# artiom-matvei/RLAO

Measured on AMD Instinct MI355X. Metric: AO env-steps/sec (batched loops), higher is better.
Workload: dtype f32; 1 GPU; 8m / 20x20 Shack-Hartmann, 256 batched envs per GPU, integrator closed loop (BASELINE.json configs[1]); envs_per_gpu=256, envs_total=256, resolution=120, n_valid_act=357, n_signal=632, layers=1, controller=leaky integrator, gain 0.5, noise=photon, parallelism=env-shards x1, all-gather of episode returns

## Files before the change

### rlao_amd/csrc/common.hpp

```cpp
#pragma once
#include <hip/hip_runtime.h>
#include <stdint.h>
#include <stddef.h>

#include <string>
#include <vector>

#include "aoenv.h"

namespace ao {

constexpr int kWave = 64;
constexpr int kMaxLayer = 8;
constexpr int kMtN = 624;
constexpr int kMaxSplits = 16;
constexpr int kMaxModes = 512;

int fail(const char* fmt, ...);
#define AO_HIP(call)                                                                          \
    do {                                                                                      \
        hipError_t e_ = (call);                                                               \
        if (e_ != hipSuccess)                                                                 \
            return ::ao::fail("%s:%d: %s -> %s", __FILE__, __LINE__, #call, hipGetErrorString(e_)); \
    } while (0)
// ... 35 lines not shown
#pragma clang fp contract(off)
    for (int d = 0; d < 2; ++d) buff[d] += fmod(fabs(ratio[d]), 1.0) * clock_sgn(ratio[d]);
    *bx = fabs(buff[0]) < 1 ? 0 : (int)clock_sgn(buff[0]);
    *by = fabs(buff[1]) < 1 ? 0 : (int)clock_sgn(buff[1]);
    for (int d = 0; d < 2; ++d) buff[d] = fmod(fabs(buff[d]), 1.0) * clock_sgn(buff[d]);
    return *bx != 0 || *by != 0;
}

__host__ __device__ inline int clock_rounds(const double ratio[2], int j, int* sx, int* sy) {
#pragma clang fp contract(off)
    const int nx = (int)fabs(ratio[0]), ny = (int)fabs(ratio[1]);
    const int mn = nx < ny ? nx : ny, mx = nx > ny ? nx : ny;
    const int s0 = (int)clock_sgn(ratio[0]), s1 = (int)clock_sgn(ratio[1]);
    if (j < mn) {
        *sx = s0;
        *sy = s1;
    } else if (j < mx) {
        *sx = nx == mn ? 0 : s0;
        *sy = ny == mn ? 0 : s1;
    } else {
        *sx = *sy = 0;
    }
    return mx;
}

__host__ __device__ inline void clock_rounds_origin(const double ratio[2], int j, int S, int org[2]) {
#pragma clang fp contract(off)
    const int nx = (int)fabs(ratio[0]), ny = (int)fabs(ratio[1]);
    const int cx = (j < nx ? j : nx) * (int)clock_sgn(ratio[0]), cy = (j < ny ? j : ny) * (int)clock_sgn(ratio[1]);
    org[0] = ((org[0] - cy) % S + S) % S;
    org[1] = ((org[1] - cx) % S + S) % S;
}

__host__ __device__ inline void taps_from_buff(const double buff[2], LayerTaps& t) {
#pragma clang fp contract(off)
    const double fy = -buff[1], fx = -buff[0];
    const double ky = floor(fy), kx = floor(fx);
    t.dy = (int)ky;
    t.dx = (int)kx;
    catmull_rom(fy - ky, t.wy);
    catmull_rom(fx - kx, t.wx);
}

struct PhaseArgs {
    const void* screen[kMaxLayer];
    const void* minmax[kMaxLayer];
    LayerTaps taps[kMaxLayer];
    int n_layer;
    int S;
    int foot;
    int S_l[kMaxLayer];
    int foot_l[kMaxLayer];
    int update_atm;
    int store_atm;
    int store_phase;
    int minmax_dirty[kMaxLayer];
    const LayerTaps* env_taps;
    int n_env;
};

__device__ inline const LayerTaps& layer_taps(const PhaseArgs& pa, int l, int e) {
    return pa.env_taps ? pa.env_taps[(size_t)l * pa.n_env + e] : pa.taps[l];
}

__device__ inline double wave_sum_f64(double v) {
    for (int off = 32; off > 0; off >>= 1) v += __shfl_down(v, off);
// ... 10 lines not shown
int launch_ring_prepare(const T* map, T* zx, const int* inner_idx, const uint32_t* mt_state, const int* mt_pos,
                        uint32_t* mt_state_out, int* mt_pos_out, const int* env_idx, int n, int S, int n_inner, int n_outer, int K,
                        int sx, int sy, int oy, int ox, const double* xi_scale, hipStream_t st);
template <typename T>
int launch_mt_normal(uint32_t* mt_state, int* mt_pos, T* zx, int n_env, int K, int n_inner, int n_outer,
                     const double* xi_scale, hipStream_t st);
template <typename T>
int launch_scatter_minmax(T* new_map, const T* X, const int* outer_idx, T* minmax, const int* env_idx, int n, int n_env, int S,
                          int n_outer, int splits, int oy, int ox, int with_minmax, hipStream_t st, const LayerTaps* env_taps = nullptr);
template <typename T>
int launch_ring_prepare_env(const T* map, T* zx, const int* inner_idx, uint32_t* mt_state, int* mt_pos, const EnvClock* clk_in,
                            EnvClock* clk_out, LayerTaps* taps, double weight, int n_env, int S, int n_inner, int n_outer, int K,
                            const double* xi_scale, hipStream_t st);
template <typename T>
int launch_ring_round_env(const T* map, T* zx, const int* inner_idx, uint32_t* mt_state, int* mt_pos, const EnvClock* clk,
                          LayerTaps* taps, int j, int n_env, int S, int n_inner, int n_outer, int K, const double* xi_scale,
                          hipStream_t st);
template <typename T>
int launch_minmax(const T* maps, T* minmax, int n_env, int S, hipStream_t st);
int launch_mt_seed(const uint32_t* seeds, int stride, const int* env_idx, uint32_t* mt_state, int* mt_pos, int n, hipStream_t st);
template <typename T>
int launch_reset_env_rows(const int* env_idx, int n_idx, T* coefs, T* dm_prev, int n_valid_act, EnvClock* clk, LayerTaps* taps,
                          int n_layer, int n_env, hipStream_t st);
int gemm_splits(int M, int N, int K);
struct MtAhead {
    const uint32_t* mt_in;
    const int* pos_in;
    uint32_t* mt_out;
    int* pos_out;
    float* zx_out;
    int K, n_inner, n_outer, n_env;
    const double* xi_scale;
};
int launch_ring_gemm_draw_ahead(const float* X, const float* W, float* Cpart, int M, int N, int K, int splits, const MtAhead& m,
                                hipStream_t st);
int launch_sum_slabs(float* x, size_t n, int slabs, hipStream_t st);
int launch_gemm_nt_mfma(const float* X, const float* W, float* Cpart, int M, int N, int K, int ldx, int ldw, int splits,
                        hipStream_t st, int xsplits = 1, size_t xslab = 0);
template <typename T>
int launch_gemm_nt(const T* X, const T* W, T* C, int M, int N, int K, int ldx, int ldw, int ldc, hipStream_t st);

__host__ __device__ inline size_t ga_index(int x, int k, int ga_stride) {
    const int q = k & 3, s = k >> 2;
    return ((((size_t)(x >> 4) * (ga_stride >> 2) + (s >> 2)) * 4 + q) * 16 + (x & 15)) * 4 + (s & 3);
}
template <typename T>
struct PhaseBuffers {
    T* opd_atm;
    const T* coefs;
    const T* coefs_img;
    const T* dm_opd;
    const T* gx;
    const T* gy;
    const T* gxt;
    const float* gxa;
    const float* gya;
    int ga_stride;
    size_t g_env, gxt_env, ga_env;
    const float* s1a;
    const int* act_idx;
    const uint8_t* pupil;
    T* phase;
    double* part;
    T* wfs_max;
};
int phase_tiles(int R, int n_act, size_t esz);
template <typename T>
int launch_coefs_image(const T* coefs, const int* act_idx, T* img, int n_env, int n_act, int n_valid_act, hipStream_t st);
// ... 68 lines not shown
                   int max_group, hipStream_t st);
struct DetectorCfg {
    int active;
    int photon_noise, bits, emccd;
    float qe, dark_e, fwc, gain, readout_noise;
    uint32_t seed_lo, seed_hi;
    uint32_t frame_counter;
    uint32_t env_offset;
};

}
#include "poisson_alias.hpp"
namespace ao {

struct StepArgs {
    KArgs<float> k;
    ShConst<float> sc;
    FinishArgs<float> fa;
    float* frame;
    int store_phase, store_frame;
    float* signal;
    float* wfs_max;
    const float* fac_m;
    const float* fac_m2c_t;
    const short* slot_of;
    const float* amp_pupil;
    const float* gxa;
    const float* gya;
    size_t ga_env;
    DetectorCfg det;
    PoissonAlias pa;
    const float* ring_x[kMaxLayer];
    int ring_splits[kMaxLayer];
    const int* outer_idx;
    int n_outer;
    float* next_zx[kMaxLayer];
    int next_sx[kMaxLayer], next_sy[kMaxLayer];
    const int* inner_idx;
    int n_inner, zx_ld;
    int n_modes, n_subap, n_valid, n_env;
};
int step_fused_supported(int R, int n_subap, int n_valid, int n_act, int n_modes);
int step_alias_capacity(int n_act);
int launch_env_step(const StepArgs& a, const StarEnv<float>& star, hipStream_t st);

template <typename T>
struct RolloutActionArgs {
    const T* obs;
    T* action;
    const T* fr;
    const T* fl_t;
    const int* act_slot;
    const T* sigma_env;
    T gain, sigma;
    int n_act, n_valid_act, n_filter;
    uint32_t seed_lo, seed_hi, counter, env_offset;
};
constexpr size_t kRolloutLdsMax = 160 * 1024;
size_t rollout_action_lds(int n_valid_act, int n_filter, size_t esz);
template <typename T>
int launch_rollout_action(const RolloutActionArgs<T>& a, int n_env, hipStream_t st);

template <typename T>
struct DisturbArgs {
    const T* coefs;
    T* seen;
// ... 142 lines not shown
```

### rlao_amd/csrc/env.hip

```cpp
#include <algorithm>
#include <cmath>
#include <cstdarg>
#include <cstdio>
#include <cstring>
#include <initializer_list>
#include <new>
#include <utility>

#include "common.hpp"
#include "delay.hpp"
#include "dm_tables.hpp"
#include "detector.hpp"
#include "disturb.hpp"
#include "modal.hpp"
#include "policy.hpp"
#include "sh_device.hpp"
#include "science.hpp"
#include "star_env.hpp"
#include "wavefront.hpp"

namespace ao {

static thread_local std::string g_err;

int fail(const char* fmt, ...) {
    char buf[1024];
    va_list ap;
    va_start(ap, fmt);
    vsnprintf(buf, sizeof(buf), fmt, ap);
    va_end(ap);
    g_err = buf;
    return 1;
}

struct LayerClock {
    double ratio[2] = {0, 0};
    double buff[2] = {0, 0};
};

struct RingAhead { bool valid = false; int sx = 0, sy = 0, buf = 0; };

struct Layer {
    int N = 0, S = 0, nin = 0, nout = 0, K = 0;
    size_t scr_off = 0;
    void* ab = nullptr;
    int* inner_idx = nullptr;
    int* outer_idx = nullptr;
    bool have_ab = false, have_in = false, have_out = false;
    double weight = 0;
    LayerClock clk;
    int org[2] = {0, 0};
    uint32_t* mt_cur = nullptr;
    int* pos_cur = nullptr;
    uint32_t* mt_alt = nullptr;
    int* pos_alt = nullptr;
    int ring_pending = 0;
    const void* ring_src = nullptr;
    RingAhead ahead;
    bool gather_next = false;
    bool minmax_dirty = false;
    int env_rounds = 0;
};

}

using namespace ao;

struct AoEnv {
    AoCfg c{};
    int device = 0;
    size_t esz = 4;
    int R = 0, A = 0, nAct = 0, E = 0, L = 0, nSig = 0, nSub = 0, nVal = 0;
    int p = 0, n = 0, n_pupil = 0;
    Layer layer[kMaxLayer];
    size_t scr_elems = 0;
    int Kmax = 0, noutmax = 0, Smax = 0;
    bool uniform = true;
    int last_zx_layer = 0;
    bool per_env_wind = false;
    EnvClock* env_clk[2] = {nullptr, nullptr};
    int clk_cur = 0;
    int wind_pixels = 1;
    LayerTaps* env_taps = nullptr;
    bool per_env_r0 = false;
    std::vector<double> h_r0;
    double* xi_scale = nullptr;
    const double* sigma() const { return per_env_r0 ? xi_scale : nullptr; }
    bool use_coefs_img = false;
    bool defer_ring = true;
    bool have[AOENV_C_COUNT] = {false};
    double units = 1.0;
    void* screen = nullptr;
    void* minmax = nullptr;
    void* zx_pipe = nullptr;
    const void* last_zx = nullptr;
    bool use_lookahead = true;
    void* zx = nullptr;
    void* xbuf = nullptr;
    void* gx = nullptr;
    void* gy = nullptr;
    void* gxt = nullptr;
    void* modes = nullptr;
    void* dm_opd = nullptr;
    int* act_idx = nullptr;
    uint8_t* pupil = nullptr;
    void* opd_atm = nullptr;
    void* coefs = nullptr;
    void* dm_prev = nullptr;
    void* coefs_seen = nullptr;
    void* step_cmd = nullptr;
    void* cmd() const { return step_cmd ? step_cmd : coefs; }
    struct Disturb {
        bool set = false;
        int M = 0, J = 0;
        int64_t t0 = 0;
        void* modes_t = nullptr;
        double* par = nullptr;
        size_t modes_cap = 0, par_cap = 0;
    } disturb;
    DelayLine delay;
    void* delay_ring = nullptr;
    size_t delay_stride = 0;
    void* delay_slot(int slot) const { return static_cast<char*>(delay_ring) + (size_t)slot * delay_stride * esz; }
    struct Modal {
        bool set = false, have_gain = false;
        int K = 0;
        size_t gain_env = 0;
// ... 94 lines not shown
    int noise_K = 0;
    std::vector<int32_t> h_act_idx;
    int* act_slot = nullptr;
    bool act_slot_dirty = true;
    void* rollout_scratch = nullptr;
    uint32_t explore_counter = 0;
    uint64_t explore_seed = 0;
    bool explore_seeded = false;
    struct Policy {
        bool set = false, mfma = false;
        int H = 0, F = 0, Kp = 0;
        double slope = 0, clamp_abs = 0, b3 = 0;
        void *w1 = nullptr, *b1 = nullptr, *w2 = nullptr, *b2 = nullptr, *w3 = nullptr, *wt1 = nullptr, *wt2 = nullptr;
        void *proj_fr = nullptr, *proj_fl_t = nullptr, *hid1 = nullptr, *hid2 = nullptr;
    } policy;
    std::vector<void*> allocs;
    bool use_fast_wfs = true;
    bool use_mfma = true;
    bool use_fast_trig = true;
    bool use_fused_tail = true;
    bool use_fused_step = true;
    bool store_opd_atm = false;
    bool atm_user_defined = false;
    int force_path = 0;
    bool prof_on = false;
    struct ProfEv { int stage; hipEvent_t a, b; };
    std::vector<ProfEv> prof_ev;

    template <typename T> T* as(void* p_) const { return static_cast<T*>(p_); }
    void* screen_ptr(int l) const { return static_cast<char*>(screen) + layer[l].scr_off * esz; }
    void* minmax_ptr(int l) const { return static_cast<char*>(minmax) + (size_t)l * E * 2 * esz; }
    void* xbuf_ptr(int l) const { return static_cast<char*>(xbuf) + (size_t)l * kMaxSplits * E * noutmax * esz; }
    void* zx_pipe_ptr(int buf, int l) const { return static_cast<char*>(zx_pipe) + ((size_t)buf * L + l) * E * Kmax * esz; }
};

namespace {

int dmalloc(AoEnv* env, void** p, size_t bytes, bool zero = true);
static int alloc_dm_rows(AoEnv* env) {
    if (env->esz == 4 && env->nAct <= 128) {
        if (!env->dm_rows)
            AO_TRY(dmalloc(env, (void**)&env->dm_rows, (size_t)env->E * (cdiv(env->R, 128) * 128) * 4 * env->ga_stride * sizeof(float)));
    } else if (!env->coefs_img) {
        AO_TRY(dmalloc(env, &env->coefs_img, (size_t)env->E * env->nAct * env->nAct * env->esz));
    }
    return 0;
}
int dmalloc(AoEnv* env, void** p, size_t bytes, bool zero) {
    if (bytes == 0) bytes = 16;
    AO_HIP(hipMalloc(p, bytes));
    env->allocs.push_back(*p);
    if (zero) AO_HIP(hipMemset(*p, 0, bytes));
    return 0;
}

struct ProfScope {
    AoEnv* env; hipStream_t st; hipEvent_t a = nullptr, b = nullptr; int stage;
    ProfScope(AoEnv* e, int stage_, hipStream_t s) : env(e), st(s), stage(stage_) {
        if (!env->prof_on) return;
        if (hipEventCreate(&a) != hipSuccess || hipEventCreate(&b) != hipSuccess) { a = b = nullptr; return; }
        (void)hipEventRecord(a, st);
    }
    ~ProfScope() {
        if (!a) return;
        (void)hipEventRecord(b, st);
        env->prof_ev.push_back({stage, a, b});
// ... 19 lines not shown
ShConst<T> sh_const(const AoEnv* env) {
    ShConst<T> sc;
    sc.amp = env->as<T>(env->amp);
    sc.subap_idx = env->subap_idx;
    sc.valid2d = env->use_fast_wfs ? env->valid2d : nullptr;
    sc.ref = env->as<T>(env->sh_ref);
    sc.tw = env->as<T>(env->tw);
    sc.ph = env->as<T>(env->phs);
    sc.units = (T)env->units;
    sc.threshold = (T)env->c.threshold_cog;
    sc.fast_trig = (env->use_fast_trig && sizeof(T) == 4) ? 1 : 0;
    sc.plain = (env->force_path & AOENV_PATH_SH_PLAIN) ? 1 : 0;
    return sc;
}

template <typename T>
int gemm_dispatch(AoEnv* env, const T* X, const T* W, T* C, int M, int N, int K, int* splits, hipStream_t st);
template <>
int gemm_dispatch<float>(AoEnv* env, const float* X, const float* W, float* C, int M, int N, int K, int* splits,
                         hipStream_t st) {
    if (!env->use_mfma) { *splits = 1; return launch_gemm_nt<float>(X, W, C, M, N, K, K, K, N, st); }
    *splits = gemm_splits(M, N, K);
    return launch_gemm_nt_mfma(X, W, C, M, N, K, K, K, *splits, st);
}
template <>
int gemm_dispatch<double>(AoEnv*, const double* X, const double* W, double* C, int M, int N, int K, int* splits,
                          hipStream_t st) {
    *splits = 1;
    return launch_gemm_nt<double>(X, W, C, M, N, K, K, K, N, st);
}

void forget_lookahead(Layer& y) { y.ahead.valid = false; y.gather_next = false; }

void drop_ring(Layer& y) { y.ring_pending = 0; }

void move_origin(Layer& y, int sx, int sy) {
    y.org[0] = ((y.org[0] - sy) % y.S + y.S) % y.S;
    y.org[1] = ((y.org[1] - sx) % y.S + y.S) % y.S;
}

void defer_ring(AoEnv* env, int l, const void* zx, int splits) {
    env->last_zx = zx;
    env->last_zx_layer = l;
    env->layer[l].ring_pending = splits;
    env->layer[l].ring_src = env->xbuf_ptr(l);
}

void take_rings(AoEnv* env, StepArgs& a) {
    for (int l = 0; l < env->L; ++l) {
        Layer& y = env->layer[l];
        a.ring_x[l] = y.ring_pending ? static_cast<const float*>(y.ring_src) : nullptr;
        a.ring_splits[l] = y.ring_pending;
        const bool g = y.gather_next && y.ring_pending && y.ahead.valid;
        a.next_zx[l] = g ? static_cast<float*>(env->zx_pipe_ptr(y.ahead.buf, l)) : nullptr;
        a.next_sx[l] = y.ahead.sx;
        a.next_sy[l] = y.ahead.sy;
        if (y.gather_next && !g) y.ahead.valid = false;
        y.gather_next = false;
    }
}

void rings_written(AoEnv* env) {
    for (int l = 0; l < env->L; ++l) { env->layer[l].ring_pending = 0; env->layer[l].minmax_dirty = false; }
}

template <typename T>
int scatter_ring(AoEnv* env, int l, const LayerTaps* et, bool with_minmax, hipStream_t st) {
    Layer& y = env->layer[l];
    AO_PROF(env, SCATTER, st);
    AO_TRY(launch_scatter_minmax<T>(env->as<T>(env->screen_ptr(l)), static_cast<const T*>(y.ring_src), y.outer_idx,
                                    env->as<T>(env->minmax_ptr(l)), nullptr, env->E, env->E, y.S, y.nout, y.ring_pending, y.org[0],
                                    y.org[1], with_minmax ? 1 : 0, st, et));
    y.ring_pending = 0;
    return 0;
}

template <typename T>
int flush_ring(AoEnv* env, int l, hipStream_t st) {
    Layer& y = env->layer[l];
    if (!y.ring_pending) return 0;
    if (y.gather_next) forget_lookahead(y);
    const LayerTaps* et = env->per_env_wind ? env->env_taps + (size_t)l * env->E : nullptr;
    return scatter_ring<T>(env, l, et, et != nullptr, st);
}
template <typename T>
int flush_rings(AoEnv* env, hipStream_t st) {
    for (int l = 0; l < env->L; ++l) AO_TRY(flush_ring<T>(env, l, st));
    return 0;
}

template <typename T>
int ring_gemm(AoEnv* env, int l, const T* zx, int* splits, hipStream_t st) {
    const Layer& y = env->layer[l];
    AO_PROF(env, GEMM_RING, st);
    return gemm_dispatch<T>(env, zx, env->as<T>(y.ab), env->as<T>(env->xbuf_ptr(l)), env->E, y.nout, y.K, splits, st);
}

template <typename T>
int extrude(AoEnv* env, int l, int sx, int sy, bool lean, hipStream_t st, bool defer = false) {
    Layer& y = env->layer[l];
    forget_lookahead(y);
    AO_TRY(flush_ring<T>(env, l, st));
    T* zx = env->as<T>(env->zx);
    {
        AO_PROF(env, SHIFT_GATHER, st);
        AO_TRY(launch_ring_prepare<T>(env->as<T>(env->screen_ptr(l)), zx, y.inner_idx, y.mt_cur, y.pos_cur, y.mt_cur, y.pos_cur, nullptr,
// ... 30 lines not shown
    if (!d_idx) y.minmax_dirty = false;
    return 0;
}

template <typename T>
int refresh_minmax(AoEnv* env, hipStream_t st) {
    AO_TRY(flush_rings<T>(env, st));
    for (int l = 0; l < env->L; ++l)
        if (env->layer[l].minmax_dirty) {
            AO_TRY(launch_minmax<T>(env->as<T>(env->screen_ptr(l)), env->as<T>(env->minmax_ptr(l)), env->E, env->layer[l].S, st));
            env->layer[l].minmax_dirty = false;
        }
    return 0;
}

bool next_crossing(const LayerClock& k0, int* sx, int* sy) {
    if ((int)std::fabs(k0.ratio[0]) > 0 || (int)std::fabs(k0.ratio[1]) > 0) return false;
    if (k0.ratio[0] == 0 && k0.ratio[1] == 0) return false;
    double b[2] = {k0.buff[0], k0.buff[1]};
    for (int it = 0; it < 1000000; ++it) {
        for (int d = 0; d < 2; ++d) b[d] += std::fmod(std::fabs(k0.ratio[d]), 1.0) * sgn(k0.ratio[d]);
        if (std::fabs(b[0]) >= 1 || std::fabs(b[1]) >= 1) {
            *sx = std::fabs(b[0]) < 1 ? 0 : (int)sgn(b[0]);
            *sy = std::fabs(b[1]) < 1 ? 0 : (int)sgn(b[1]);
            return true;
        }
        for (int d = 0; d < 2; ++d) b[d] = std::fmod(std::fabs(b[d]), 1.0) * sgn(b[d]);
    }
    return false;
}

int extrude_pipelined(AoEnv* env, int l, int sx, int sy, hipStream_t st) {
    Layer& y = env->layer[l];
    const int cur = y.ahead.buf;
    float* op = static_cast<float*>(env->zx_pipe_ptr(cur, l));
    if (y.ahead.valid && y.ahead.sx == sx && y.ahead.sy == sy) {
        std::swap(y.mt_cur, y.mt_alt);
        std::swap(y.pos_cur, y.pos_alt);
    } else {
        AO_PROF(env, SHIFT_GATHER, st);
        AO_TRY(launch_ring_prepare<float>(env->as<float>(env->screen_ptr(l)), op, y.inner_idx, y.mt_cur, y.pos_cur, y.mt_cur, y.pos_cur,
                                          nullptr, env->E, y.S, y.nin, y.nout, y.K, sx, sy, y.org[0], y.org[1], env->sigma(), st));
    }
    forget_lookahead(y);
    const int splits = gemm_splits(env->E, y.nout, y.K);
    MtAhead m{y.mt_cur, y.pos_cur, y.mt_alt, y.pos_alt, static_cast<float*>(env->zx_pipe_ptr(1 - cur, l)), y.K, y.nin, y.nout, env->E,
              env->sigma()};
    {
        AO_PROF(env, GEMM_RING, st);
        AO_TRY(launch_ring_gemm_draw_ahead(op, env->as<float>(y.ab), static_cast<float*>(env->xbuf_ptr(l)), env->E, y.nout, y.K, splits, m,
                                           st));
    }
    move_origin(y, sx, sy);
    defer_ring(env, l, op, splits);
    y.minmax_dirty = true;
    int nsx = 0, nsy = 0;
    if (next_crossing(y.clk, &nsx, &nsy)) {
        y.ahead = RingAhead{true, nsx, nsy, 1 - cur};
        y.gather_next = true;
    }
    return 0;
}

template <typename T>
int advance_atmosphere_env(AoEnv* env, bool lean, hipStream_t st) {
    for (int l = 0; l < env->L; ++l) {
        AO_TRY(flush_ring<T>(env, l, st));
        const Layer& y = env->layer[l];
        T* zx = env->as<T>(env->zx);
        const size_t row = (size_t)l * env->E;
        for (int j = 0; j < y.env_rounds; ++j) {
            {
                AO_PROF(env, SHIFT_GATHER, st);
                AO_TRY(launch_ring_round_env<T>(env->as<T>(env->screen_ptr(l)), zx, y.inner_idx, y.mt_cur, y.pos_cur,
                                                env->env_clk[env->clk_cur] + row, env->env_taps + row, j, env->E, y.S, y.nin, y.nout,
                                                y.K, env->sigma(), st));
            }
            int splits = 1;
            AO_TRY(ring_gemm<T>(env, l, zx, &splits, st));
            defer_ring(env, l, zx, splits);
            AO_TRY(flush_ring<T>(env, l, st));
        }
        {
            AO_PROF(env, SHIFT_GATHER, st);
            AO_TRY(launch_ring_prepare_env<T>(env->as<T>(env->screen_ptr(l)), zx, y.inner_idx, y.mt_cur, y.pos_cur,
                                              env->env_clk[env->clk_cur] + row, env->env_clk[1 - env->clk_cur] + row, env->env_taps + row,
                                              y.weight, env->E, y.S, y.nin, y.nout, y.K, env->sigma(), st));
// ... 719 lines not shown

    AoEnv* e = new (std::nothrow) AoEnv();
    if (!e) return fail("out of host memory");
    e->c = *cfg;
    e->device = device;
    e->esz = cfg->dtype == AOENV_F32 ? 4 : 8;
    e->R = cfg->resolution; e->A = cfg->n_valid_act; e->nAct = cfg->n_act; e->E = cfg->n_env; e->L = cfg->n_layer;
    e->nSig = cfg->n_signal; e->nSub = cfg->n_subap; e->nVal = cfg->n_valid_subap;
    e->p = e->R / e->nSub; e->n = 2 * e->p;
    e->layer[0].N = cfg->layer_res;
    e->layer[0].S = cfg->layer_res + 2;
    for (int l = 0; l < e->L; ++l) {
        Layer& y = e->layer[l];
        y.N = cfg->layer_res_l[l] ? cfg->layer_res_l[l] : cfg->layer_res;
        y.S = y.N + 2;
        y.nin = 8 * y.N - 16;
        y.nout = 4 * y.N + 4;
        y.K = y.nin + y.nout;
        y.scr_off = e->scr_elems;
        e->scr_elems += (size_t)e->E * y.S * y.S;
        e->Kmax = std::max(e->Kmax, y.K);
        e->noutmax = std::max(e->noutmax, y.nout);
        e->Smax = std::max(e->Smax, y.S);
        if (y.N != e->layer[0].N) e->uniform = false;
    }
    const size_t z = e->esz, E = e->E, R2 = (size_t)e->R * e->R;
    int rc = 0;
    auto A_ = [&](void** p, size_t bytes) { if (!rc) rc = dmalloc(e, p, bytes); };
    if (e->L > 0) {
        A_(&e->screen, e->scr_elems * z);
        A_(&e->minmax, (size_t)e->L * E * 2 * z);
        if (cfg->dtype == AOENV_F32) {
            A_(&e->zx_pipe, (size_t)2 * e->L * E * e->Kmax * z);
        }
        A_(&e->zx, E * e->Kmax * z);
        A_(&e->xbuf, (size_t)e->L * kMaxSplits * E * e->noutmax * z);
        for (int l = 0; l < e->L; ++l) {
            Layer& y = e->layer[l];
            A_((void**)&y.mt_cur, E * kMtN * 4);
            A_((void**)&y.pos_cur, E * 4);
            A_((void**)&y.mt_alt, E * kMtN * 4);
            A_((void**)&y.pos_alt, E * 4);
            if (l > 0 && e->uniform) {
                y.ab = e->layer[0].ab;
                y.inner_idx = e->layer[0].inner_idx;
                y.outer_idx = e->layer[0].outer_idx;
                continue;
            }
            A_(&y.ab, (size_t)y.nout * y.K * z);
            A_((void**)&y.inner_idx, (size_t)y.nin * 4);
            A_((void**)&y.outer_idx, (size_t)y.nout * 4);
        }
    }
    A_(&e->gx, (size_t)e->R * e->nAct * z);
    A_(&e->gy, (size_t)e->R * e->nAct * z);
    A_(&e->gxt, (size_t)((e->nAct + 3) & ~3) * (size_t)(cdiv(e->R, 128) * 128) * z);
    if (!cfg->dm_separable) {
        A_(&e->modes, R2 * e->A * z);
        A_(&e->dm_opd, E * R2 * z);
    }
    A_((void**)&e->act_idx, (size_t)e->A * 4);
    A_((void**)&e->pupil, R2);
    A_(&e->opd_atm, E * R2 * z);
    A_(&e->coefs, E * e->A * z);
    A_(&e->coefs_seen, E * e->A * z);
    A_(&e->dm_prev, E * e->A * z);
// ... 1989 lines not shown
```

### rlao_amd/csrc/gemm_kernels.hip

```cpp
#include "common.hpp"
#include "ring_device.hpp"

namespace ao {

template <typename T>
__global__ void __launch_bounds__(256) k_gemm_nt(const T* __restrict__ X, const T* __restrict__ W, T* __restrict__ C,
                                                 int M, int N, int K, int ldx, int ldw, int ldc) {
    constexpr int BM = 64, BN = 64, BK = 16;
    __shared__ T xs[BK][BM + 1];
    __shared__ T ws[BK][BN + 1];
    const int m0 = blockIdx.y * BM, n0 = blockIdx.x * BN;
    const int tx = threadIdx.x % 16, ty = threadIdx.x / 16;
    T acc[4][4];
#pragma unroll
    for (int i = 0; i < 4; ++i)
#pragma unroll
        for (int j = 0; j < 4; ++j) acc[i][j] = (T)0;

    for (int k0 = 0; k0 < K; k0 += BK) {
        for (int q = threadIdx.x; q < BM * BK; q += 256) {
            const int r = q / BK, kk = q % BK;
            const int gm = m0 + r, gn = n0 + r, gk = k0 + kk;
            xs[kk][r] = (gm < M && gk < K) ? X[(size_t)gm * ldx + gk] : (T)0;
            ws[kk][r] = (gn < N && gk < K) ? W[(size_t)gn * ldw + gk] : (T)0;
// ... 91 lines not shown
            float* xd = xs + r * LDT + kq;
            float* wd = ws + r * LDT + kq;
            xd[0] = xv[pass].x; xd[1] = xv[pass].y; xd[2] = xv[pass].z; xd[3] = xv[pass].w;
            wd[0] = wv[pass].x; wd[1] = wv[pass].y; wd[2] = wv[pass].z; wd[3] = wv[pass].w;
        }
        __syncthreads();
        if (k0 + BK < kend) fetch(k0 + BK);
        const float* xa = xs + (wm + lr) * LDT + lh;
        const float* wb = ws + (wn + lr) * LDT + lh;
#pragma unroll
        for (int kk = 0; kk < BK / 2; ++kk)
            acc = __builtin_amdgcn_mfma_f32_32x32x2f32(xa[2 * kk], wb[2 * kk], acc, 0, 0, 0);
        __syncthreads();
    }
    float* C = Cpart + (size_t)bz * M * N;
    const int gn = n0 + wn + lr;
    if (gn < N) {
#pragma unroll
        for (int rg = 0; rg < 16; ++rg) {
            const int gm = m0 + wm + (rg & 3) + 8 * (rg >> 2) + 4 * lh;
            if (gm < M) C[(size_t)gm * N + gn] = acc[rg];
        }
    }
}

__global__ void __launch_bounds__(256) k_gemm_nt_mfma(const float* __restrict__ X, const float* __restrict__ W,
                                                      float* __restrict__ Cpart, int M, int N, int K, int ldx,
                                                      int ldw, int kslice, int xsplits, size_t xslab) {
    gemm_nt_mfma_tile(X, W, Cpart, M, N, K, ldx, ldw, kslice, xsplits, xslab, (int)blockIdx.z);
}

__global__ void __launch_bounds__(256) k_ring_gemm_draw_ahead(const float* __restrict__ X, const float* __restrict__ W,
                                                              float* __restrict__ Cpart, int M, int N, int K, int ldx, int ldw,
                                                              int kslice, int splits, const MtAhead m) {
    const int draw_slices = (int)gridDim.z - splits;
    if ((int)blockIdx.z >= draw_slices) {
        gemm_nt_mfma_tile(X, W, Cpart, M, N, K, ldx, ldw, kslice, 1, 0, (int)blockIdx.z - draw_slices);
        return;
    }
    const int e = ((int)blockIdx.z * (int)gridDim.y + (int)blockIdx.y) * (int)gridDim.x + (int)blockIdx.x;
    if (e < m.n_env) mt_normal_body<float>(m.mt_in, m.pos_in, m.mt_out, m.pos_out, m.zx_out, m.K, m.n_inner, m.n_outer, e,
                                           m.xi_scale);
}

int launch_ring_gemm_draw_ahead(const float* X, const float* W, float* Cpart, int M, int N, int K, int splits, const MtAhead& m,
                                hipStream_t st) {
    if (m.n_outer % 2) return fail("mt_normal: n_outer=%d must be even", m.n_outer);
    const int kslice = cdiv(cdiv(K, splits), 32) * 32;
    const int gx = cdiv(N, 64), gy = cdiv(M, 64);
    dim3 grid(gx, gy, splits + cdiv(m.n_env, gx * gy));
    hipLaunchKernelGGL(k_ring_gemm_draw_ahead, grid, dim3(256), 0, st, X, W, Cpart, M, N, K, K, K, kslice, splits, m);
    AO_HIP(hipGetLastError());
    return 0;
}

int gemm_splits(int M, int N, int K) {
    const int tiles = cdiv(M, 64) * cdiv(N, 64);
    if (K > 2048) {
        int best = 1;
        double best_cost = 1e300;
        for (int s = 1; s <= kMaxSplits; ++s) {
            const int wgs = tiles * s, kslice = cdiv(cdiv(K, s), 32) * 32;
            if (wgs < 1024 && s < kMaxSplits && tiles * (s + 1) <= 1024) continue;
            const double cost = (double)cdiv(wgs, 256) * (kslice + 96) + (double)s * M * N * 8.0 / 4e12 / 20e-9;
            if (cost < best_cost) { best_cost = cost; best = s; }
        }
        return best;
    }
    (void)tiles;
    const int smax = K / 64 > 0 ? K / 64 : 1;
    return smax > kMaxSplits ? kMaxSplits : smax;
}

__global__ void __launch_bounds__(256) k_sum_slabs(float* __restrict__ x, int n4, int slabs, size_t slab4) {
    const int i = blockIdx.x * 256 + threadIdx.x;
    if (i >= n4) return;
    float4* p = reinterpret_cast<float4*>(x);
    float4 v[kMaxSplits];
#pragma unroll
    for (int z = 0; z < kMaxSplits; ++z) v[z] = p[(size_t)(z < slabs ? z : 0) * slab4 + i];
    float4 a = v[0];
#pragma unroll
    for (int z = 1; z < kMaxSplits; ++z)
        if (z < slabs) { a.x += v[z].x; a.y += v[z].y; a.z += v[z].z; a.w += v[z].w; }
// ... 124 lines not shown
```

### rlao_amd/csrc/ring_device.hpp

```cpp
#pragma once
#include "common.hpp"

namespace ao {

__device__ inline int torus(int r, int c, int oy, int ox, int S) {
    int pr = r + oy, pc = c + ox;
    pr = pr >= S ? pr - S : pr;
    pc = pc >= S ? pc - S : pc;
    return pr * S + pc;
}

template <typename T>
__device__ inline void gather_ring(const T* __restrict__ map, T* __restrict__ zx, const int* __restrict__ inner_idx, int S,
                                   int n_inner, int K, int sx, int sy, int oy, int ox, int e, int t0, int nt) {
    const T* src = map + (size_t)e * S * S;
    for (int k = t0; k < n_inner; k += nt) {
        const int idx = inner_idx[k];
        const int r = idx / S - sy, c = idx % S - sx;
        zx[(size_t)e * K + k] = src[torus(r, c, oy, ox, S)];
    }
}

__device__ inline uint32_t mt_temper(uint32_t y) {
    y ^= (y >> 11);
    y ^= (y << 7) & 0x9d2c5680u;
    y ^= (y << 15) & 0xefc60000u;
    y ^= (y >> 18);
    return y;
}

__device__ inline uint32_t mt_mix(uint32_t a, uint32_t b, uint32_t far) {
    uint32_t y = (a & 0x80000000u) | (b & 0x7fffffffu);
    return far ^ (y >> 1) ^ ((y & 1u) ? 0x9908b0dfu : 0u);
}

constexpr int kMtTry = kMtN / 4;
constexpr int kMtSlots = 4;
constexpr int kMtLaneTry = 2 * 256;

__device__ inline void mt_twist_next(const uint32_t* s, uint32_t* n) {
    const int t = threadIdx.x;
    if (t < 227) n[t] = mt_mix(s[t], s[t + 1], s[t + 397]);
    __syncthreads();
    if (t < 227) n[t + 227] = mt_mix(s[t + 227], s[t + 228], n[t]);
    __syncthreads();
    if (t < 169) n[t + 454] = mt_mix(s[t + 454], s[t + 455], n[t + 227]);
    if (t == 192) n[623] = mt_mix(s[623], n[0], n[396]);
    __syncthreads();
}

__device__ inline bool mt_polar(const uint32_t* w, double& n0, double& n1) {
#pragma clang fp contract(off)
    const double d1 = ((double)(mt_temper(w[0]) >> 5) * 67108864.0 + (double)(mt_temper(w[1]) >> 6)) /
                      9007199254740992.0;
    const double d2 = ((double)(mt_temper(w[2]) >> 5) * 67108864.0 + (double)(mt_temper(w[3]) >> 6)) /
                      9007199254740992.0;
    const double x1 = 2.0 * d1 - 1.0, x2 = 2.0 * d2 - 1.0;
    const double r2 = x1 * x1 + x2 * x2;
    if (!(r2 < 1.0 && r2 != 0.0)) return false;
    const double f = sqrt(-2.0 * log(r2) / r2);
    n0 = f * x2;
    n1 = f * x1;
    return true;
}

template <typename T>
__device__ inline void mt_normal_body(const uint32_t* mt_state, const int* mt_pos, uint32_t* mt_state_out, int* mt_pos_out,
                                      T* __restrict__ zx, int K, int n_inner, int n_outer, int e, const double* xi_scale) {
    __shared__ uint32_t s[kMtSlots * kMtN];
    __shared__ int scan[4];
    __shared__ int sh_stop;
    const int t = threadIdx.x;
    const int lane = t & (kWave - 1), wv = t / kWave;
    const uint32_t* gs = mt_state + (size_t)e * kMtN;
    uint32_t* gso = mt_state_out + (size_t)e * kMtN;
    for (int i = t; i < kMtN; i += 256) s[i] = gs[i];
    int pos = mt_pos[e], got = 0, cur = 0;
    const double sg = xi_scale ? xi_scale[e] : 1.0;
    __syncthreads();
    const int need_pairs = n_outer / 2;
    T* out = zx + (size_t)e * K + n_inner;
    auto slot = [](int b) { return b >= kMtSlots ? b - kMtSlots : b; };
    while (got < need_pairs) {
        const int remaining = need_pairs - got;
        const int avail0 = (kMtN - pos) / 4;
        const int want = remaining + remaining / 3 + 16 - avail0;
        const int nt = want <= 0 ? 0 : min((kMtLaneTry - avail0) / kMtTry, (want + kMtTry - 1) / kMtTry);
        for (int j = 0; j < nt; ++j) mt_twist_next(s + slot(cur + j) * kMtN, s + slot(cur + j + 1) * kMtN);
        const int n_try = avail0 + kMtTry * nt;
        bool acc[2];
        double n0[2], n1[2];
#pragma unroll
        for (int u = 0; u < 2; ++u) {
            const int a = 2 * t + u;
            acc[u] = false;
            n0[u] = n1[u] = 0.0;
            if (a < n_try) {
                const int a2 = a - avail0;
                const uint32_t* w = a2 < 0 ? s + cur * kMtN + pos + 4 * a
                                           : s + slot(cur + 1 + a2 / kMtTry) * kMtN + 4 * (a2 % kMtTry);
                acc[u] = mt_polar(w, n0[u], n1[u]);
                if (acc[u] && xi_scale) {
// ... 12 lines not shown
        for (int q = 0; q < wv; ++q) before += scan[q];
        const int total_acc = scan[0] + scan[1] + scan[2] + scan[3];
#pragma unroll
        for (int u = 0; u < 2; ++u) {
            before += acc[u] ? 1 : 0;
            if (acc[u] && before <= remaining) {
                const int j = got + before - 1;
                out[2 * j] = (T)n0[u];
                out[2 * j + 1] = (T)n1[u];
                if (before == remaining) sh_stop = 2 * t + u;
            }
        }
        __syncthreads();
        const int stop = sh_stop;
        if (stop >= 0) {
            const int a2 = stop - avail0;
            if (a2 < 0) pos += 4 * (stop + 1);
            else {
                cur = slot(cur + 1 + a2 / kMtTry);
                pos = 4 * (a2 % kMtTry + 1);
            }
            got = need_pairs;
        } else {
            cur = slot(cur + nt);
            pos = kMtN;
            got += total_acc;
        }
        __syncthreads();
    }
    for (int i = t; i < kMtN; i += 256) gso[i] = s[cur * kMtN + i];
    if (t == 0) mt_pos_out[e] = pos;
}

}
```

### rlao_amd/csrc/step_kernel_body.hpp

```cpp
#pragma once
#include "step_kernel.hpp"

#include "phase_device.hpp"
#include "sh_device.hpp"
#include "detector.hpp"
#include "ring_device.hpp"

#include "camera_sh6.hpp"


namespace ao {

typedef float f32x4s __attribute__((ext_vector_type(4)));

template <typename P>
__device__ inline float ld_or0(const P* __restrict__ p, long idx, bool ok) {
    const float v = (float)p[ok ? idx : 0];
    return ok ? v : 0.f;
}

template <bool PE>
__device__ inline const LayerTaps& step_taps(const PhaseArgs& pa, int l, int e) {
    if constexpr (PE) return pa.env_taps[(size_t)l * pa.n_env + e];
    else return pa.taps[l];
// ... 18 lines not shown
    short* slot_s = reinterpret_cast<short*>(lds + L.slot);
    cplx<float>* E0 = reinterpret_cast<cplx<float>*>(lds + L.e0);
    float* sl = lds + L.sl;
    float* img_s = lds + L.img;
    const uint32_t* tab_s = reinterpret_cast<const uint32_t*>(lds + L.tab);
    __shared__ double red[4][16];
    __shared__ double red_tail[16];
    __shared__ float red_mx[16];

    const int e = blockIdx.x;
    const int tid = threadIdx.x, w = tid >> 6, lane = tid & 63;
    const int lc = lane & 15, lq = lane >> 4;
    const int band = w >> 2, cg = w & 3;
    const size_t pix0 = (size_t)e * R * R;
    const int n_sub = a.n_subap, n_valid = a.n_valid;

    const float ctab = fast6::cos_table_lane<float>();
    f32x4s gx_raw[2][2], gy_raw[2];
#pragma unroll
    for (int tt = 0; tt < 2; ++tt) {
        const f32x4s* src = reinterpret_cast<const f32x4s*>(a.gxa + e * a.ga_env) + (2 * cg + tt) * 2 * 64 + (tid & 63);
        gx_raw[tt][0] = src[0];
        gx_raw[tt][1] = src[64];
    }
    const int rt = w >> 1, ct = w & 1;
    {
        const f32x4s* src = reinterpret_cast<const f32x4s*>(a.gya + e * a.ga_env) + rt * 2 * 64 + (tid & 63);
        gy_raw[0] = src[0];
        gy_raw[1] = src[64];
    }
    float mm_pre[kMaxLayer];
#pragma unroll
    for (int l = 0; l < kMaxLayer; ++l)
        mm_pre[l] = l < k.pa.n_layer ? static_cast<const float*>(k.pa.minmax[l])[2 * e + (tid & 1)] : 0.f;
    const bool has_act = tid < k.n_valid_act;
    const int act_px = k.pb.act_idx[has_act ? tid : 0];
    const float act_c = k.pb.coefs[(size_t)e * k.n_valid_act + (has_act ? tid : 0)];
    const short slot_v = a.slot_of[tid < n_sub * n_sub ? tid : 0];
    for (int i = tid; i < nA * nA; i += 1024) cimg[i] = 0.f;
    for (int i = tid; i < 2 * PR * SS; i += 1024) s1[i] = 0.f;
    if (tid < n_sub * n_sub) slot_s[tid] = slot_v;
    for (int i = tid + 1024; i < n_sub * n_sub; i += 1024) slot_s[i] = a.slot_of[i];
    lds_barrier();
    if (has_act) cimg[act_px] = act_c;
    float breg[2][KS];
#pragma unroll
    for (int tt = 0; tt < 2; ++tt) {
        const float t[8] = {gx_raw[tt][0][0], gx_raw[tt][0][1], gx_raw[tt][0][2], gx_raw[tt][0][3],
                            gx_raw[tt][1][0], gx_raw[tt][1][1], gx_raw[tt][1][2], gx_raw[tt][1][3]};
#pragma unroll
        for (int ks = 0; ks < KS; ++ks) breg[tt][ks] = t[ks];
    }

    lds_barrier();
    {
        const int ix = 16 * ct + lc;
        float av[KS], bv[KS];
        {
            const float t[8] = {gy_raw[0][0], gy_raw[0][1], gy_raw[0][2], gy_raw[0][3], gy_raw[1][0], gy_raw[1][1], gy_raw[1][2], gy_raw[1][3]};
#pragma unroll
            for (int ks = 0; ks < KS; ++ks) av[ks] = t[ks];
        }
#pragma unroll
        for (int ks = 0; ks < KS; ++ks) {
            const int iy = lq + 4 * ks;
            bv[ks] = ld_or0(cimg, iy * nA + ix, iy < nA && ix < nA);
        }
        f32x4s d = {0.f, 0.f, 0.f, 0.f};
#pragma unroll
        for (int ks = 0; ks < KS; ++ks) d = __builtin_amdgcn_mfma_f32_16x16x4f32(av[ks], bv[ks], d, 0, 0, 0);
        if (ix < nA) {
#pragma unroll
            for (int r = 0; r < 4; ++r) s1[(16 * rt + 4 * lq + r) * SS + ix] = d[r];
        }
    }

    {
        bool any = false;
        for (int l = 0; l < k.pa.n_layer; ++l) {
            const float* x = a.ring_x[l];
            if (x == nullptr) continue;
            any = true;
            const LayerTaps& tl = step_taps<PE>(k.pa, l, e);
            if (PE && !tl.ring) continue;
            float* map = const_cast<float*>(static_cast<const float*>(k.pa.screen[l])) + (size_t)e * S * S;
            const size_t slab = (size_t)a.n_env * a.n_outer;
            const int oy = tl.oy, ox = tl.ox;
            for (int q = tid; q < a.n_outer; q += 1024) {
                float xv[kMaxSplits];
#pragma unroll
                for (int z = 0; z < kMaxSplits; ++z)
                    xv[z] = x[(size_t)(z < a.ring_splits[l] ? z : 0) * slab + (size_t)e * a.n_outer + q];
                float v = xv[0];
#pragma unroll
                for (int z = 1; z < kMaxSplits; ++z) v += z < a.ring_splits[l] ? xv[z] : 0.f;
                const int idx = a.outer_idx[q];
                int pr = idx / S + oy, pc = idx % S + ox;
                pr = pr >= S ? pr - S : pr;
                pc = pc >= S ? pc - S : pc;
                map[pr * S + pc] = v;
            }
        }
        if (any) __syncthreads();
        if (!PE) {
            for (int l = 0; l < k.pa.n_layer; ++l)
                if (a.next_zx[l] != nullptr)
                    gather_ring<float>(static_cast<const float*>(k.pa.screen[l]), a.next_zx[l], a.inner_idx, S, a.n_inner, a.zx_ld,
                                       a.next_sx[l], a.next_sy[l], k.pa.taps[l].oy, k.pa.taps[l].ox, e, tid, 1024);
        }
    }

    __shared__ float lohi[kMaxLayer][2];
    __shared__ float red_lo[16], red_hi[16];
    for (int l = 0; l < k.pa.n_layer; ++l) {
        float* mm = const_cast<float*>(static_cast<const float*>(k.pa.minmax[l])) + 2 * e;
        const bool dirty = k.pa.minmax_dirty[l] || (PE && a.ring_x[l] != nullptr && step_taps<PE>(k.pa, l, e).ring);
        if (!dirty) {
            float pre = 0.f;
#pragma unroll
            for (int q = 0; q < kMaxLayer; ++q) pre = q == l ? mm_pre[q] : pre;
            if (tid < 2) lohi[l][tid] = pre;
            continue;
        }
        const float* map = static_cast<const float*>(k.pa.screen[l]) + (size_t)e * S * S;
        const int n4 = (S * S) / 4;
        float lo = 3.0e38f, hi = -3.0e38f;
        if ((S * S) % 4 == 0) {
            for (int i0 = tid; i0 < n4; i0 += 4 * 1024) {
                f32x4s v[4];
#pragma unroll
                for (int u = 0; u < 4; ++u) v[u] = *reinterpret_cast<const f32x4s*>(map + 4 * (i0 + 1024 * u < n4 ? i0 + 1024 * u : i0));
#pragma unroll
                for (int u = 0; u < 4; ++u)
#pragma unroll
                    for (int d = 0; d < 4; ++d) { lo = v[u][d] < lo ? v[u][d] : lo; hi = v[u][d] > hi ? v[u][d] : hi; }
            }
        } else {
            for (int i = tid; i < S * S; i += 1024) { const float v = map[i]; lo = v < lo ? v : lo; hi = v > hi ? v : hi; }
        }
        for (int off = 32; off > 0; off >>= 1) {
            const float ol = __shfl_down(lo, off), oh = __shfl_down(hi, off);
            lo = ol < lo ? ol : lo;
            hi = oh > hi ? oh : hi;
        }
        lds_barrier();
        if (lane == 0) { red_lo[w] = lo; red_hi[w] = hi; }
        lds_barrier();
        if (tid == 0) {
            for (int i = 1; i < 16; ++i) { lo = red_lo[i] < lo ? red_lo[i] : lo; hi = red_hi[i] > hi ? red_hi[i] : hi; }
            lohi[l][0] = lo; lohi[l][1] = hi;
            mm[0] = lo; mm[1] = hi;
        }
    }

    PupilSums sums;
// ... 333 lines not shown
```

Measured before the change: 5.730 million env-steps/s.

## Compute phase-screen min/max from interior range plus scattered ring values

Instead of rescanning the whole phase-screen map for min/max after each ring extrusion, the ring GEMM launch adds extra blocks that compute the min/max of the torus interior (excluding the border rows and columns about to be overwritten). The step kernel then combines that with a warp reduction over the newly scattered ring values. This avoids a full-map reduction inside the latency-critical step kernel, at the cost of extra blocks in the GEMM launch, a new buffer, and a fallback when either bound is exactly zero.

```diff
diff --git a/rlao_amd/csrc/common.hpp b/rlao_amd/csrc/common.hpp
--- a/rlao_amd/csrc/common.hpp
+++ b/rlao_amd/csrc/common.hpp
@@ -91,6 +91,11 @@
     org[1] = ((org[1] - cx) % S + S) % S;
 }
 
+__host__ __device__ inline bool torus_border(int pr, int pc, int oy, int ox, int S) {
+    const int ly = oy == 0 ? S - 1 : oy - 1, lx = ox == 0 ? S - 1 : ox - 1;
+    return pr == oy || pr == ly || pc == ox || pc == lx;
+}
+
 __host__ __device__ inline void taps_from_buff(const double buff[2], LayerTaps& t) {
 #pragma clang fp contract(off)
     const double fy = -buff[1], fx = -buff[0];
@@ -167,8 +172,13 @@
     int K, n_inner, n_outer, n_env;
     const double* xi_scale;
 };
+struct RingRange {
+    const float* map;
+    float* mm;
+    int S, oy, ox;
+};
 int launch_ring_gemm_draw_ahead(const float* X, const float* W, float* Cpart, int M, int N, int K, int splits, const MtAhead& m,
-                                hipStream_t st);
+                                const RingRange& rr, hipStream_t st);
 int launch_sum_slabs(float* x, size_t n, int slabs, hipStream_t st);
 int launch_gemm_nt_mfma(const float* X, const float* W, float* Cpart, int M, int N, int K, int ldx, int ldw, int splits,
                         hipStream_t st, int xsplits = 1, size_t xslab = 0);
@@ -303,6 +313,7 @@
     PoissonAlias pa;
     const float* ring_x[kMaxLayer];
     int ring_splits[kMaxLayer];
+    const float* ring_mm[kMaxLayer];
     const int* outer_idx;
     int n_outer;
     float* next_zx[kMaxLayer];
diff --git a/rlao_amd/csrc/env.hip b/rlao_amd/csrc/env.hip
--- a/rlao_amd/csrc/env.hip
+++ b/rlao_amd/csrc/env.hip
@@ -56,6 +56,7 @@
     int* pos_alt = nullptr;
     int ring_pending = 0;
     const void* ring_src = nullptr;
+    bool ring_ranged = false;
     RingAhead ahead;
     bool gather_next = false;
     bool minmax_dirty = false;
@@ -93,6 +94,7 @@
     void* screen = nullptr;
     void* minmax = nullptr;
     void* zx_pipe = nullptr;
+    void* ring_mm = nullptr;
     const void* last_zx = nullptr;
     bool use_lookahead = true;
     void* zx = nullptr;
@@ -253,6 +255,7 @@
     void* minmax_ptr(int l) const { return static_cast<char*>(minmax) + (size_t)l * E * 2 * esz; }
     void* xbuf_ptr(int l) const { return static_cast<char*>(xbuf) + (size_t)l * kMaxSplits * E * noutmax * esz; }
     void* zx_pipe_ptr(int buf, int l) const { return static_cast<char*>(zx_pipe) + ((size_t)buf * L + l) * E * Kmax * esz; }
+    float* ring_mm_ptr(int l) const { return static_cast<float*>(ring_mm) + (size_t)l * E * 2; }
 };
 
 namespace {
@@ -338,18 +341,20 @@
 
 void forget_lookahead(Layer& y) { y.ahead.valid = false; y.gather_next = false; }
 
-void drop_ring(Layer& y) { y.ring_pending = 0; }
-
-void move_origin(Layer& y, int sx, int sy) {
-    y.org[0] = ((y.org[0] - sy) % y.S + y.S) % y.S;
-    y.org[1] = ((y.org[1] - sx) % y.S + y.S) % y.S;
-}
+void drop_ring(Layer& y) { y.ring_pending = 0; y.ring_ranged = false; }
+
+void moved_origin(const Layer& y, int sx, int sy, int org[2]) {
+    org[0] = ((y.org[0] - sy) % y.S + y.S) % y.S;
+    org[1] = ((y.org[1] - sx) % y.S + y.S) % y.S;
+}
+void move_origin(Layer& y, int sx, int sy) { moved_origin(y, sx, sy, y.org); }
 
 void defer_ring(AoEnv* env, int l, const void* zx, int splits) {
     env->last_zx = zx;
     env->last_zx_layer = l;
     env->layer[l].ring_pending = splits;
     env->layer[l].ring_src = env->xbuf_ptr(l);
+    env->layer[l].ring_ranged = false;
 }
 
 void take_rings(AoEnv* env, StepArgs& a) {
@@ -357,6 +362,7 @@
         Layer& y = env->layer[l];
         a.ring_x[l] = y.ring_pending ? static_cast<const float*>(y.ring_src) : nullptr;
         a.ring_splits[l] = y.ring_pending;
+        a.ring_mm[l] = y.ring_pending && y.ring_ranged ? env->ring_mm_ptr(l) : nullptr;
         const bool g = y.gather_next && y.ring_pending && y.ahead.valid;
         a.next_zx[l] = g ? static_cast<float*>(env->zx_pipe_ptr(y.ahead.buf, l)) : nullptr;
         a.next_sx[l] = y.ahead.sx;
@@ -367,7 +373,7 @@
 }
 
 void rings_written(AoEnv* env) {
-    for (int l = 0; l < env->L; ++l) { env->layer[l].ring_pending = 0; env->layer[l].minmax_dirty = false; }
+    for (int l = 0; l < env->L; ++l) { drop_ring(env->layer[l]); env->layer[l].minmax_dirty = false; }
 }
 
 template <typename T>
@@ -377,7 +383,7 @@
     AO_TRY(launch_scatter_minmax<T>(env->as<T>(env->screen_ptr(l)), static_cast<const T*>(y.ring_src), y.outer_idx,
                                     env->as<T>(env->minmax_ptr(l)), nullptr, env->E, env->E, y.S, y.nout, y.ring_pending, y.org[0],
                                     y.org[1], with_minmax ? 1 : 0, st, et));
-    y.ring_pending = 0;
+    drop_ring(y);
     return 0;
 }
 
@@ -474,6 +480,7 @@
 
 int extrude_pipelined(AoEnv* env, int l, int sx, int sy, hipStream_t st) {
     Layer& y = env->layer[l];
+    if (y.ring_pending) return fail("extrude_pipelined: layer %d has a ring pending", l);
     const int cur = y.ahead.buf;
     float* op = static_cast<float*>(env->zx_pipe_ptr(cur, l));
     if (y.ahead.valid && y.ahead.sx == sx && y.ahead.sy == sy) {
@@ -488,13 +495,17 @@
     const int splits = gemm_splits(env->E, y.nout, y.K);
     MtAhead m{y.mt_cur, y.pos_cur, y.mt_alt, y.pos_alt, static_cast<float*>(env->zx_pipe_ptr(1 - cur, l)), y.K, y.nin, y.nout, env->E,
               env->sigma()};
+    int org[2];
+    moved_origin(y, sx, sy, org);
+    const RingRange rr{env->as<float>(env->screen_ptr(l)), env->ring_mm_ptr(l), y.S, org[0], org[1]};
     {
         AO_PROF(env, GEMM_RING, st);
         AO_TRY(launch_ring_gemm_draw_ahead(op, env->as<float>(y.ab), static_cast<float*>(env->xbuf_ptr(l)), env->E, y.nout, y.K, splits, m,
-                                           st));
+                                           rr, st));
     }
     move_origin(y, sx, sy);
     defer_ring(env, l, op, splits);
+    y.ring_ranged = true;
     y.minmax_dirty = true;
     int nsx = 0, nsy = 0;
     if (next_crossing(y.clk, &nsx, &nsy)) {
@@ -1280,6 +1291,7 @@
         A_(&e->minmax, (size_t)e->L * E * 2 * z);
         if (cfg->dtype == AOENV_F32) {
             A_(&e->zx_pipe, (size_t)2 * e->L * E * e->Kmax * z);
+            A_(&e->ring_mm, (size_t)e->L * E * 2 * sizeof(float));
         }
         A_(&e->zx, E * e->Kmax * z);
         A_(&e->xbuf, (size_t)e->L * kMaxSplits * E * e->noutmax * z);
diff --git a/rlao_amd/csrc/gemm_kernels.hip b/rlao_amd/csrc/gemm_kernels.hip
--- a/rlao_amd/csrc/gemm_kernels.hip
+++ b/rlao_amd/csrc/gemm_kernels.hip
@@ -147,24 +147,30 @@
 
 __global__ void __launch_bounds__(256) k_ring_gemm_draw_ahead(const float* __restrict__ X, const float* __restrict__ W,
                                                               float* __restrict__ Cpart, int M, int N, int K, int ldx, int ldw,
-                                                              int kslice, int splits, const MtAhead m) {
-    const int draw_slices = (int)gridDim.z - splits;
-    if ((int)blockIdx.z >= draw_slices) {
-        gemm_nt_mfma_tile(X, W, Cpart, M, N, K, ldx, ldw, kslice, 1, 0, (int)blockIdx.z - draw_slices);
+                                                              int kslice, int splits, int env_slices, const MtAhead m,
+                                                              const RingRange rr) {
+    const int z = (int)blockIdx.z;
+    const int p0 = (int)gridDim.z - splits;
+    if (z >= p0) {
+        gemm_nt_mfma_tile(X, W, Cpart, M, N, K, ldx, ldw, kslice, 1, 0, z - p0);
         return;
     }
-    const int e = ((int)blockIdx.z * (int)gridDim.y + (int)blockIdx.y) * (int)gridDim.x + (int)blockIdx.x;
-    if (e < m.n_env) mt_normal_body<float>(m.mt_in, m.pos_in, m.mt_out, m.pos_out, m.zx_out, m.K, m.n_inner, m.n_outer, e,
-                                           m.xi_scale);
+    const bool draw = z < env_slices;
+    const int e = ((draw ? z : z - env_slices) * (int)gridDim.y + (int)blockIdx.y) * (int)gridDim.x + (int)blockIdx.x;
+    if (e >= m.n_env) return;
+    if (draw) mt_normal_body<float>(m.mt_in, m.pos_in, m.mt_out, m.pos_out, m.zx_out, m.K, m.n_inner, m.n_outer, e, m.xi_scale);
+    else ring_interior_range(rr, e);
 }
 
 int launch_ring_gemm_draw_ahead(const float* X, const float* W, float* Cpart, int M, int N, int K, int splits, const MtAhead& m,
-                                hipStream_t st) {
+                                const RingRange& rr, hipStream_t st) {
     if (m.n_outer % 2) return fail("mt_normal: n_outer=%d must be even", m.n_outer);
+    if (rr.map && (rr.oy < 0 || rr.oy >= rr.S || rr.ox < 0 || rr.ox >= rr.S)) return fail("ring range: origin (%d, %d) outside the %d-torus", rr.oy, rr.ox, rr.S);
     const int kslice = cdiv(cdiv(K, splits), 32) * 32;
     const int gx = cdiv(N, 64), gy = cdiv(M, 64);
-    dim3 grid(gx, gy, splits + cdiv(m.n_env, gx * gy));
-    hipLaunchKernelGGL(k_ring_gemm_draw_ahead, grid, dim3(256), 0, st, X, W, Cpart, M, N, K, K, K, kslice, splits, m);
+    const int env_slices = cdiv(m.n_env, gx * gy);
+    dim3 grid(gx, gy, splits + env_slices * (rr.map ? 2 : 1));
+    hipLaunchKernelGGL(k_ring_gemm_draw_ahead, grid, dim3(256), 0, st, X, W, Cpart, M, N, K, K, K, kslice, splits, env_slices, m, rr);
     AO_HIP(hipGetLastError());
     return 0;
 }
diff --git a/rlao_amd/csrc/ring_device.hpp b/rlao_amd/csrc/ring_device.hpp
--- a/rlao_amd/csrc/ring_device.hpp
+++ b/rlao_amd/csrc/ring_device.hpp
@@ -37,6 +37,11 @@
 constexpr int kMtTry = kMtN / 4;
 constexpr int kMtSlots = 4;
 constexpr int kMtLaneTry = 2 * 256;
+
+__device__ inline uint32_t* mt_state_lds() {
+    __shared__ uint32_t s[kMtSlots * kMtN];
+    return s;
+}
 
 __device__ inline void mt_twist_next(const uint32_t* s, uint32_t* n) {
     const int t = threadIdx.x;
@@ -67,7 +72,7 @@
 template <typename T>
 __device__ inline void mt_normal_body(const uint32_t* mt_state, const int* mt_pos, uint32_t* mt_state_out, int* mt_pos_out,
                                       T* __restrict__ zx, int K, int n_inner, int n_outer, int e, const double* xi_scale) {
-    __shared__ uint32_t s[kMtSlots * kMtN];
+    uint32_t* s = mt_state_lds();
     __shared__ int scan[4];
     __shared__ int sh_stop;
     const int t = threadIdx.x;
@@ -146,4 +151,72 @@
     if (t == 0) mt_pos_out[e] = pos;
 }
 
-}
+__device__ inline void ring_interior_range(const RingRange& rr, int e) {
+    float* red = reinterpret_cast<float*>(mt_state_lds());
+    const int t = threadIdx.x, S = rr.S, n = S * S;
+    const float* map = rr.map + (size_t)e * n;
+    const int mis = (int)((reinterpret_cast<uintptr_t>(map) >> 2) & 3);
+    const int h = min((4 - mis) & 3, n);
+    const int n4 = (n - h) / 4, tail = h + 4 * n4;
+    const float4* m4 = reinterpret_cast<const float4*>(map + h);
+    float lo = 3.0e38f, hi = -3.0e38f;
+    auto fold = [&](float v, bool in) {
+        lo = (in && v < lo) ? v : lo;
+        hi = (in && v > hi) ? v : hi;
+    };
+    const int dq = 1024 / S, dr = 1024 - dq * S;
+    int pr = (h + 4 * t) / S, pc = (h + 4 * t) - pr * S;
+    for (int i0 = t; i0 < n4; i0 += 8 * 256) {
+        float4 v[8];
+#pragma unroll
+        for (int q = 0; q < 8; ++q) {
+            const int i = i0 + 256 * q;
+            v[q] = m4[i < n4 ? i : i0];
+        }
+#pragma unroll
+        for (int q = 0; q < 8; ++q) {
+            const int i = i0 + 256 * q;
+            const bool ok = i < n4;
+            int r = pr, c = pc;
+            const float f[4] = {v[q].x, v[q].y, v[q].z, v[q].w};
+#pragma unroll
+            for (int d = 0; d < 4; ++d) {
+                fold(f[d], ok && !torus_border(r, c, rr.oy, rr.ox, S));
+                if (++c == S) { c = 0; ++r; }
+            }
+            pr += dq;
+            pc += dr;
+            if (pc >= S) { pc -= S; ++pr; }
+        }
+    }
+    {
+        const int k = t & 3;
+        const int j = t < 4 ? k : tail + k;
+        const bool ok = t < 8 && (t < 4 ? k < h : j < n);
+        const int jc = ok ? j : 0;
+        const float v = map[jc];
+        const int er = jc / S, ec = jc - er * S;
+        fold(v, ok && !torus_border(er, ec, rr.oy, rr.ox, S));
+    }
+    for (int off = 32; off > 0; off >>= 1) {
+        const float ol = __shfl_down(lo, off), oh = __shfl_down(hi, off);
+        lo = ol < lo ? ol : lo;
+        hi = oh > hi ? oh : hi;
+    }
+    const int w = t / kWave;
+    if ((t & (kWave - 1)) == 0) {
+        red[w] = lo;
+        red[4 + w] = hi;
+    }
+    __syncthreads();
+    if (t == 0) {
+        for (int i = 1; i < 4; ++i) {
+            lo = red[i] < lo ? red[i] : lo;
+            hi = red[4 + i] > hi ? red[4 + i] : hi;
+        }
+        rr.mm[2 * e] = lo;
+        rr.mm[2 * e + 1] = hi;
+    }
+}
+
+}
diff --git a/rlao_amd/csrc/step_kernel_body.hpp b/rlao_amd/csrc/step_kernel_body.hpp
--- a/rlao_amd/csrc/step_kernel_body.hpp
+++ b/rlao_amd/csrc/step_kernel_body.hpp
@@ -74,7 +74,7 @@
     float mm_pre[kMaxLayer];
 #pragma unroll
     for (int l = 0; l < kMaxLayer; ++l)
-        mm_pre[l] = l < k.pa.n_layer ? static_cast<const float*>(k.pa.minmax[l])[2 * e + (tid & 1)] : 0.f;
+        mm_pre[l] = l < k.pa.n_layer ? static_cast<const float*>(!PE && a.ring_mm[l] ? a.ring_mm[l] : k.pa.minmax[l])[2 * e + (tid & 1)] : 0.f;
     const bool has_act = tid < k.n_valid_act;
     const int act_px = k.pb.act_idx[has_act ? tid : 0];
     const float act_c = k.pb.coefs[(size_t)e * k.n_valid_act + (has_act ? tid : 0)];
@@ -117,6 +117,8 @@
         }
     }
 
+    constexpr int kRangeSlots = 4;
+    float* red_rng = reinterpret_cast<float*>(&red[0][0]);
     {
         bool any = false;
         for (int l = 0; l < k.pa.n_layer; ++l) {
@@ -128,6 +130,7 @@
             float* map = const_cast<float*>(static_cast<const float*>(k.pa.screen[l])) + (size_t)e * S * S;
             const size_t slab = (size_t)a.n_env * a.n_outer;
             const int oy = tl.oy, ox = tl.ox;
+            float rlo = 3.0e38f, rhi = -3.0e38f;
             for (int q = tid; q < a.n_outer; q += 1024) {
                 float xv[kMaxSplits];
 #pragma unroll
@@ -141,6 +144,16 @@
                 pr = pr >= S ? pr - S : pr;
                 pc = pc >= S ? pc - S : pc;
                 map[pr * S + pc] = v;
+                rlo = v < rlo ? v : rlo;
+                rhi = v > rhi ? v : rhi;
+            }
+            if (!PE && l < kRangeSlots) {
+                for (int off = 32; off > 0; off >>= 1) {
+                    const float ol = __shfl_down(rlo, off), oh = __shfl_down(rhi, off);
+                    rlo = ol < rlo ? ol : rlo;
+                    rhi = oh > rhi ? oh : rhi;
+                }
+                if (lane == 0) { red_rng[32 * l + w] = rlo; red_rng[32 * l + 16 + w] = rhi; }
             }
         }
         if (any) __syncthreads();
@@ -163,6 +176,31 @@
             for (int q = 0; q < kMaxLayer; ++q) pre = q == l ? mm_pre[q] : pre;
             if (tid < 2) lohi[l][tid] = pre;
             continue;
+        }
+        if (!PE && l < kRangeSlots && a.ring_mm[l] != nullptr) {
+            float lo = red_rng[32 * l + (lane & 15)], hi = red_rng[32 * l + 16 + (lane & 15)];
+            {
+                float pre = 0.f;
+#pragma unroll
+                for (int q = 0; q < kRangeSlots; ++q) pre = q == l ? mm_pre[q] : pre;
+                const float plo = __shfl(pre, 0), phi = __shfl(pre, 1);
+                lo = plo < lo ? plo : lo;
+                hi = phi > hi ? phi : hi;
+            }
+            for (int off = 8; off > 0; off >>= 1) {
+                const float ol = __shfl_xor(lo, off), oh = __shfl_xor(hi, off);
+                lo = ol < lo ? ol : lo;
+                hi = oh > hi ? oh : hi;
+            }
+            lo = __builtin_bit_cast(float, __builtin_amdgcn_readfirstlane(__builtin_bit_cast(int, lo)));
+            hi = __builtin_bit_cast(float, __builtin_amdgcn_readfirstlane(__builtin_bit_cast(int, hi)));
+            if (lo != 0.f && hi != 0.f) {
+                if (tid == 0) {
+                    lohi[l][0] = lo; lohi[l][1] = hi;
+                    mm[0] = lo; mm[1] = hi;
+                }
+                continue;
+            }
         }
         const float* map = static_cast<const float*>(k.pa.screen[l]) + (size_t)e * S * S;
         const int n4 = (S * S) / 4;
```

Measured after the change: 5.756 million env-steps/s (median of 6 runs). Within noise of the previous version (+0.5%).
